# ChantalMP/RaDialog

Hardware: AMD Instinct MI355X
Metric: reports_per_sec (448px CXR encode + 160-tok prefill + 256-tok greedy decode) (higher is better)
Workload: dtype bf16; 1 GPU; configs[1]: per-GPU batch 1 BioViL-T(ResNet-50)+Q-Former encode 448px, Vicuna-7B prefill T=160, 256-token greedy decode (LoRA r=8 un-merged, hipGraph ; per_gpu_batch=1, global_batch=1, prompt_len=160, parallelism=dp1

## Files before the change

### radialog_amd/csrc/api.hip

```cpp
#include "rdx_ctx.h"

static std::string g_create_err;

int fail(rdx_ctx* c, int code, const char* fmt, ...) {
    char buf[512];
    va_list ap;
    va_start(ap, fmt);
    vsnprintf(buf, sizeof(buf), fmt, ap);
    va_end(ap);
    if (c) c->err = buf; else g_create_err = buf;
    return code;
}

const char* create_error() { return g_create_err.c_str(); }

int dalloc(rdx_ctx* c, void** p, size_t bytes) {
    if (bytes == 0) bytes = 16;
    hipError_t e = hipMalloc(p, bytes);
    if (e != hipSuccess) return fail(c, -3, "hipMalloc(%zu bytes) failed: %s", bytes, hipGetErrorString(e));
    c->allocs.push_back(*p);
    return 0;
}

extern "C" int rdx_create(rdx_ctx** out, int device_id, const rdx_config* cfg) {
// ... 4 lines not shown
    if (e != hipSuccess || ndev <= 0) return fail(nullptr, -2, "rdx_create: no HIP device (%s)", hipGetErrorString(e));
    if (device_id < 0 || device_id >= ndev) return fail(nullptr, -1, "rdx_create: device %d out of range (%d devices)", device_id, ndev);
    if (cfg->enable_llama) {
        if (cfg->hidden % cfg->heads || cfg->hidden / cfg->heads != 128)
            return fail(nullptr, -1, "rdx_create: Llama head_dim must be 128 (hidden %d / heads %d)", cfg->hidden, cfg->heads);
        if (cfg->hidden % 32 || cfg->inter % 32 || cfg->inter % 8 || cfg->qformer_dim % 32)
            return fail(nullptr, -1, "rdx_create: hidden/inter/qformer_dim must be multiples of 32");
        if (cfg->max_len % 32 || cfg->max_len <= 0 || cfg->max_len > 1536)
            return fail(nullptr, -1, "rdx_create: max_len must be a multiple of 32 in (0, 1536]");
        if (cfg->max_batch <= 0 || cfg->max_batch > RDX_MAX_ROWS) return fail(nullptr, -1, "rdx_create: max_batch must be in [1, %d]", RDX_MAX_ROWS);
        if (cfg->lora_r != 0 && cfg->lora_r != 8) return fail(nullptr, -1, "rdx_create: lora_r must be 0 or 8");
    }
    if (cfg->enable_vision) {
        if (cfg->q_hidden / cfg->q_heads != 64 || cfg->q_hidden % cfg->q_heads)
            return fail(nullptr, -1, "rdx_create: Q-Former head_dim must be 64");
    }
    if (cfg->enable_vision || cfg->enable_cls) {
        if (cfg->v_img % 4 || cfg->v_img < 32) return fail(nullptr, -1, "rdx_create: image size must be a multiple of 4, >= 32");
    }
    if (cfg->enable_cls) {
        if (cfg->enable_vision) return fail(nullptr, -1, "rdx_create: a classifier context has enable_vision = 0 (its projector differs)");
        if (cfg->cls_pool <= 0 || cfg->cls_hidden % 32 || cfg->cls_classes <= 0 || cfg->cls_classes > 16)
            return fail(nullptr, -1, "rdx_create: classifier needs pool > 0, hidden %% 32 == 0, 1..16 classes");
    }
    rdx_ctx* c = new rdx_ctx();
    c->cfg = *cfg;
    c->device = device_id;
    if (const char* e = getenv("RDX_FUSE_AO")) c->fuse_attn_oproj = atoi(e) != 0;
    if (const char* e = getenv("RDX_CHAIN")) c->chain_mlp = atoi(e) != 0;
    if (hipSetDevice(device_id) != hipSuccess || hipStreamCreateWithFlags(&c->stream, hipStreamNonBlocking) != hipSuccess) {
        delete c;
        return fail(nullptr, -2, "rdx_create: cannot create stream on device %d", device_id);
    }
    { const char* e = getenv("RDX_FLASH_MIN"); if (e) c->flash_min = atoi(e); }
    { const char* e = getenv("RDX_XS16"); if (e) c->xs16 = atoi(e) != 0; }
    { const char* e = getenv("RDX_PBLK"); if (e) c->prompt_blk = atoi(e) != 0; }
    { const char* e = getenv("RDX_BLK_DOWN"); c->blk_down = !(e && atoi(e) == 0); }
    { const char* e = getenv("RDX_PCONV_KSPLIT"); c->pconv_noks = e && atoi(e) == 0; }
    { const char* e = getenv("RDX_PCONV"); c->trunk_packed = !(e && atoi(e) == 0); }
    if (hipMalloc(&c->zero16, 64) == hipSuccess) { hipMemset(c->zero16, 0, 64); c->allocs.push_back(c->zero16); } else c->zero16 = nullptr;
    c->gemm_ws_floats = (size_t)16 << 20;
    if (hipMalloc((void**)&c->gemm_ws, c->gemm_ws_floats * sizeof(float)) != hipSuccess) { c->gemm_ws = nullptr; c->gemm_ws_floats = 0; }
    else c->allocs.push_back(c->gemm_ws);
    *out = c;
    return 0;
}

void rdx_comm_release(rdx_ctx* c);

extern "C" void rdx_destroy(rdx_ctx* c) {
    if (!c) return;
    hipSetDevice(c->device);
    hipStreamSynchronize(c->stream);
    rdx_comm_release(c);
    if (c->graph) hipGraphExecDestroy(c->graph);
    for (void* p : c->allocs) hipFree(p);
    hipStreamDestroy(c->stream);
    delete c;
}

extern "C" const char* rdx_last_error(rdx_ctx* c) { return c ? c->err.c_str() : g_create_err.c_str(); }

#ifndef RDX_BUILD_HASH
#define RDX_BUILD_HASH "unstamped"
#endif
extern "C" const char* rdx_build_hash(void) { return RDX_BUILD_HASH; }
// ... 230 lines not shown
        if (c->tens.count("v.pool.emb")) {
            const int Cv = f.v_b2v, Pn = v_grid(f) * v_grid(f);
            if (Cv % 32) return fail(c, -1, "ViT pooler needs b2v %% 32 == 0");
            c->pool_emb = R.t("v.pool.emb", (int64_t)2 * Pn * Cv);
            c->pool_ng = R.f("v.pool.norm_g", Cv); c->pool_nb = R.f("v.pool.norm_b", Cv);
            c->v_p1f = R.g("v.proj1f.w", f.v_proj, 2 * Cv); c->v_p1f_b = R.f("v.proj1f.b", f.v_proj);
            for (int i = 0; c->gemm.count(S("v.pool.%d.wqkv", i)); ++i) {
                PoolBlock pb;
                const std::string p = S("v.pool.%d.", i);
                pb.n1_g = R.f(p + "n1_g", Cv); pb.n1_b = R.f(p + "n1_b", Cv); pb.n2_g = R.f(p + "n2_g", Cv); pb.n2_b = R.f(p + "n2_b", Cv);
                pb.wqkv = R.g(p + "wqkv", 3 * Cv, Cv);
                pb.wo = R.g(p + "wo", Cv, Cv); pb.bo = R.f(p + "bo", Cv);
                pb.w1 = R.g(p + "w1", Cv, Cv); pb.b1 = R.f(p + "b1", Cv);
                pb.w2 = R.g(p + "w2", Cv, Cv); pb.b2 = R.f(p + "b2", Cv);
                c->pool.push_back(pb);
            }
        }
    }
    if (R.rc) return R.rc;
    c->finalized = true;
    return 0;
}

extern "C" int rdx_set_option(rdx_ctx* c, const char* name, int value) {
    if (!c || !name) return -1;
    if (!strcmp(name, "flash_min")) { c->flash_min = value; return 0; }
    if (!strcmp(name, "pconv")) { c->trunk_packed = value != 0; return 0; }
    if (!strcmp(name, "prompt_blk")) { c->prompt_blk = value != 0; return 0; }
    if (!strcmp(name, "xs16")) {
        c->xs16 = value != 0;
        if (c->graph) { hipGraphExecDestroy(c->graph); c->graph = nullptr; c->gkey = GraphKey(); }
        return 0;
    }
    return fail(c, -1, "rdx_set_option: unknown option '%s'", name);
}
```

### radialog_amd/csrc/api_debug.hip

```cpp
#include "rdx_ctx.h"
#include "../../include/rdx_hooks.h"
#include "../../include/rdx_enc_hooks.h"

extern "C" int rdx_attn_trace(rdx_ctx* c, int layer, long long* host) {
    if (!c || !c->finalized || c->cur_B <= 0 || !host) return fail(c, -1, "rdx_attn_trace: run a prefill first");
    HIPCHK(c, hipSetDevice(c->device));
    long long* dtr = nullptr;
    HIPCHK(c, hipMalloc(&dtr, 8 * sizeof(long long)));
    HIPCHK(c, hipMemsetAsync(dtr, 0, 8 * sizeof(long long), c->stream));
    DecAttnArgs at = dec_attn_args(c, layer);
    at.trace = dtr;
    launch_decode_attention(c->cfg.dtype, at, c->cur_B, c->stream);
    hipError_t e = hipStreamSynchronize(c->stream);
    if (e == hipSuccess) e = hipMemcpy(host, dtr, 8 * sizeof(long long), hipMemcpyDeviceToHost);
    hipFree(dtr);
    HIPCHK(c, e);
    return 0;
}

extern "C" int rdx_quant_test(rdx_ctx* c, const void* X, int M, int K, int groups, int mode, const void* norm_w, float eps, void* out8, float* scales) {
    if (!c || !X || !out8 || !scales || M <= 0 || K <= 0 || K % 128) return fail(c, -1, "rdx_quant_test: bad arguments (K %% 128 == 0)");
    if (mode == 0 && (groups < 1 || groups > 4)) return fail(c, -1, "rdx_quant_test: 1..4 K groups");
    if (mode == 1 && !norm_w) return fail(c, -1, "rdx_quant_test: mode 1 needs the norm weight");
    HIPCHK(c, hipSetDevice(c->device));
    if (mode == 0) launch_quant_rows(c->cfg.dtype, X, K, out8, scales, M, K, groups, c->stream);
    else launch_rmsnorm_fp8(c->cfg.dtype, X, norm_w, out8, scales, M, K, eps, c->stream);
    HIPCHK(c, hipStreamSynchronize(c->stream));
    HIPCHK(c, hipGetLastError());
    return 0;
}

extern "C" int rdx_gemv_trace(rdx_ctx* c, int what, int layer, long long* host, int max_tiles) {
    if (!c || !c->finalized || c->cur_B <= 0 || !host) return fail(c, -1, "rdx_gemv_trace: run a prefill first");
    HIPCHK(c, hipSetDevice(c->device));
    const rdx_config& f = c->cfg;
    const int H = f.hidden, B = c->cur_B;
    if (what == 7) {
        if (layer < 0 || layer >= f.layers) return fail(c, -1, "rdx_gemv_trace(7): layer %d of %d", layer, f.layers);
        if (c->cur_T + c->cur_steps + 1 > f.max_len || c->cur_T + c->cur_steps + 1 > f.max_pos)
            return fail(c, -1, "rdx_gemv_trace(7): no room for one more decode step in the KV cache");
        const int wgs = H / 16 + ((c->ll[0].wqkv.Npad + 15) / 16 + 3) / 4;
        if (wgs > max_tiles) return fail(c, -1, "rdx_gemv_trace(7): need room for %d workgroups", wgs);
        long long* dtr = nullptr;
        const size_t bytes = (size_t)max_tiles * 8 * sizeof(long long);
        HIPCHK(c, hipMalloc(&dtr, bytes));
        HIPCHK(c, hipMemsetAsync(dtr, 0, bytes, c->stream));
        c->chain_trace = dtr; c->chain_trace_layer = layer;
        const bool chained = decode_step_launch(c, nullptr, nullptr, 0);
        c->chain_trace = nullptr; c->chain_trace_layer = -1;
        c->cur_steps = std::max(c->cur_steps + 1, c->cur_max_new);
        hipError_t e = hipStreamSynchronize(c->stream);
        if (e == hipSuccess) e = hipMemcpy(host, dtr, bytes, hipMemcpyDeviceToHost);
        hipFree(dtr);
        HIPCHK(c, e);
        if (!chained) return fail(c, -1, "rdx_gemv_trace(7): the chained down -> QKV launch is not active in this configuration (batch > 2, RDX_CHAIN=0)");
        return 0;
    }
    const LlamaLayer& L = c->ll[layer];
    long long* dtr = nullptr;
    const size_t bytes = (size_t)max_tiles * 8 * sizeof(long long);
    HIPCHK(c, hipMalloc(&dtr, bytes));
    HIPCHK(c, hipMemsetAsync(dtr, 0, bytes, c->stream));
    GemmArgs a = unit_args(c, &L, what == 1 ? UNIT_GATE_UP : what == 2 ? UNIT_QKV : UNIT_DOWN, B);
    if (what != 1 && what != 2) { a.out = c->dqkv; a.resid = nullptr; a.ldr = 0; }
    if ((a.N + 15) / 16 > max_tiles) { hipFree(dtr); return fail(c, -1, "rdx_gemv_trace: need room for %d tiles", (a.N + 15) / 16); }
    a.trace = dtr;
    skinny(c, a, what == 1 ? EPI_SILU_MUL : EPI_NONE);
    hipError_t e = hipStreamSynchronize(c->stream);
    if (e == hipSuccess) e = hipMemcpy(host, dtr, bytes, hipMemcpyDeviceToHost);
// ... 464 lines not shown
```

### radialog_amd/csrc/api_llama.hip

```cpp
#include "rdx_ctx.h"

static int ensure_prefill_ws(rdx_ctx* c, size_t rows) {
    rows = (rows + 15) & ~(size_t)15;
    if (rows <= c->prefill_rows) return 0;
    const rdx_config& f = c->cfg;
    HIPCHK(c, hipStreamSynchronize(c->stream));
    c->prefill_rows = 0;
    dfree(c, c->px); dfree(c, c->pxn); dfree(c, c->pqkv); dfree(c, c->pq); dfree(c, c->patt); dfree(c, c->pgu); dfree(c, c->pxq); dfree(c, c->pxs); dfree(c, c->pslab);
    if (fp8_weights(c->ll[0].wqkv)) {
        ALLOC(c, c->pxq, rows * (size_t)std::max(f.hidden, f.inter));
        ALLOC(c, c->pxs, rows * 4 * sizeof(float));
    }
    ALLOC(c, c->px, rows * f.hidden * 2); ALLOC(c, c->pxn, rows * f.hidden * 2);
    ALLOC(c, c->pslab, (size_t)4 * std::min<size_t>(rows, 192) * f.hidden * sizeof(float));
    ALLOC(c, c->pqkv, rows * c->ld.qkv_ld * 2); ALLOC(c, c->pq, rows * f.hidden * 2);
    ALLOC(c, c->patt, rows * f.hidden * 2); ALLOC(c, c->pgu, rows * f.inter * 2);
    c->prefill_rows = rows;
    return 0;
}

static const char* const k_need_blk = "more than 32 decoder rows need hidden 4096 / inter 11008 (the row-block family)";

static void lm_head_and_greedy(rdx_ctx* c, const void* x, int B, void* logits, const int* out_step, long step_stride,
                               int advance) {
// ... 164 lines not shown
    for (int l = 0; l < c->cfg.layers; ++l) {
        const LlamaLayer* L = &c->ll[l];
        launch_xstat_blk8(dt, norm_in_front(c, blk8_unit(c, L, UNIT_QKV, B)), EPI_NONE, s);
        DecAttnArgs at = dec_attn_args(c, l);
        at.out_packed = 2;
        launch_decode_attention(dt, at, B, s);
        ksplit(blk8_unit(c, L, UNIT_O, B));
        launch_xstat_blk8(dt, norm_in_front(c, blk8_unit(c, L, UNIT_GATE_UP, B)), EPI_SILU_MUL, s);
        ksplit(blk8_unit(c, L, UNIT_DOWN, B));
    }
}

static void step_xs16(rdx_ctx* c, int B) {
    const int dt = c->cfg.dtype;
    hipStream_t s = c->stream;
    for (int l = 0; l < c->cfg.layers; ++l) {
        const LlamaLayer* L = &c->ll[l];
        launch_xstat16(dt, xs16_unit(c, L, UNIT_QKV, B), EPI_NONE, s);
        DecAttnArgs at = dec_attn_args(c, l);
        at.out_packed = 1;
        launch_decode_attention(dt, at, B, s);
        launch_xrow16(dt, xs16_unit(c, L, UNIT_O, B), s);
        launch_xstat16(dt, xs16_unit(c, L, UNIT_GATE_UP, B), EPI_SILU_MUL, s);
        launch_xrow16(dt, xs16_unit(c, L, UNIT_DOWN, B), s);
    }
}

static void attn_oproj(rdx_ctx* c, int l, int B) {
    const int dt = c->cfg.dtype;
    const LlamaLayer& L = c->ll[l];
    DecAttnArgs at = dec_attn_args(c, l);
    const GemmArgs ao = unit_args(c, &L, UNIT_O, B);
    if (c->fuse_attn_oproj && attn_oproj16_supported(c->ld, L.wo.N, L.wo.K, B)) {
        launch_attn_oproj16(dt, at, ao, B, c->d_ctr + (size_t)l * 256, c->d_err, c->stream);
        return;
    }
    const GemmArgs ap = ksplit_args(ao);
    const int kg = (B >= xs_min_rows() && c->kslab) ? xsplit32_groups(ap) : 0;
    at.out_packed = kg > 0 ? ap.xpacked : 0;
    launch_decode_attention(dt, at, B, c->stream);
    if (kg) launch_ksplit(c, ap);
    else skinny(c, ao, EPI_RESID);
}

static void step_generic(rdx_ctx* c, int B) {
    for (int l = 0; l < c->cfg.layers; ++l) {
        const LlamaLayer& L = c->ll[l];
        skinny(c, unit_args(c, &L, UNIT_QKV, B), EPI_NONE);
        attn_oproj(c, l, B);
        const bool split = down_split_ok(c, L, B);
        GemmArgs gu = unit_args(c, &L, UNIT_GATE_UP, B);
        gu.out_packed = split ? ksplit_args(unit_args(c, &L, UNIT_DOWN, B)).xpacked : 0;
        skinny(c, gu, EPI_SILU_MUL);
        launch_down(c, L, B, split);
    }
}

static void step_chained(rdx_ctx* c, int B, std::vector<hipEvent_t>* evs) {
    const rdx_config& f = c->cfg;
    hipStream_t s = c->stream;
    ChainArgs ca;
    memset(&ca, 0, sizeof(ca));
    ca.layers = c->d_clayers; ca.hidden = f.hidden; ca.inter = f.inter; ca.qkv_n = c->ll[0].wqkv.Npad; ca.qkv_ld = c->ld.qkv_ld; ca.B = B; ca.eps = f.rms_eps;
    ca.dx = c->dx; ca.dqkv = c->dqkv; ca.dgu = c->dgu; ca.ctr = c->d_cctr; ca.err = c->d_err; ca.naps = c->chain_naps;
    const LlamaLayer& L0 = c->ll[0];
    ca.w8 = (L0.wqkv.w8 && L0.wdown.w8 && f.hidden % 64 == 0 && f.inter % 64 == 0) ? 1 : 0;
    auto mark = [&] { if (evs) { hipEvent_t e; hipEventCreate(&e); hipEventRecord(e, s); evs->push_back(e); } };
    skinny(c, unit_args(c, &L0, UNIT_QKV, B), EPI_NONE);
    for (int l = 0; l < f.layers; ++l) {
        attn_oproj(c, l, B);
        skinny(c, unit_args(c, &c->ll[l], UNIT_GATE_UP, B), EPI_SILU_MUL);
        mark();
        ca.layer = l;
        ca.trace = l == c->chain_trace_layer ? c->chain_trace : nullptr;
        launch_decode_chain(f.dtype, ca, l + 1 < f.layers, s);
        mark();
    }
}

bool decode_step_launch(rdx_ctx* c, void* logits, const int* out_step, long step_stride, std::vector<hipEvent_t>* evs) {
    const int B = c->cur_B;
    const DecFamily fam = decode_family(c, B);
    switch (fam) {
    case DEC_UNSUPPORTED: c->unsupported = k_need_blk; return false;
    case DEC_BLK: step_blk(c, B); break;
    case DEC_BLK8: step_blk8(c, B); break;
    case DEC_XS16: step_xs16(c, B); break;
    case DEC_CHAINED: step_chained(c, B, evs); break;
    case DEC_GENERIC: step_generic(c, B); break;
    }
    lm_head_and_greedy(c, c->dx, B, logits, out_step, step_stride, 1);
    return fam == DEC_CHAINED;
}

extern "C" int rdx_decode_step(rdx_ctx* c, void* logits) {
    if (!c) return -1;
    if (!c->finalized || c->cur_B <= 0) return fail(c, -1, "rdx_decode_step: no prefill has run");
    if (c->cur_steps >= c->cur_max_new)
        return fail(c, -1, "rdx_decode_step: all %d tokens of this prompt (max_new) have been generated; run a new prefill", c->cur_max_new);
    if (c->cur_T + c->cur_steps > c->cfg.max_len || c->cur_T + c->cur_steps > c->cfg.max_pos)
        return fail(c, -1, "rdx_decode_step: KV cache full (%d prompt + %d generated slots of %d)", c->cur_T, c->cur_steps, c->cfg.max_len);
    HIPCHK(c, hipSetDevice(c->device));
    decode_step_launch(c, logits, nullptr, 0);
    ++c->cur_steps;
// ... 246 lines not shown
```

### radialog_amd/csrc/attn_body.h

```cpp
#pragma once
#include "rdx_common.h"
#include "rdx_kernels.h"
#include "handoff.h"

namespace rdx {

template <typename T>
__device__ __forceinline__ float rope_one(float x, float partner_signed, float c, float s) {
    return rnd<T>(rnd<T>(x * c) + rnd<T>(partner_signed * s));
}

__host__ __device__ inline size_t decode_attention_smem_floats(int waves, int max_len) { return (size_t)waves * 128 + 128 + max_len; }

template <int N> __device__ __forceinline__ float row_share(float v) { return dpp_mov<0x150 + N>(v); }

template <typename T> __device__ __forceinline__ float dot2(unsigned a, unsigned b, float c);
template <> __device__ __forceinline__ float dot2<bf16>(unsigned a, unsigned b, float c) {
    typedef __bf16 v2b __attribute__((ext_vector_type(2)));
    return __builtin_amdgcn_fdot2_f32_bf16(__builtin_bit_cast(v2b, a), __builtin_bit_cast(v2b, b), c, false);
}
template <> __device__ __forceinline__ float dot2<f16>(unsigned a, unsigned b, float c) {
    typedef _Float16 v2h __attribute__((ext_vector_type(2)));
    return __builtin_amdgcn_fdot2(__builtin_bit_cast(v2h, a), __builtin_bit_cast(v2h, b), c, false);
}

template <typename T, int WAVES, bool DED = (WAVES == 8), typename WaitFn = NoWait, bool V_EARLY_ = !DED, int KG_ = 0, bool COH = false>
__device__ __forceinline__ void decode_attention_body(const DecAttnArgs& a, const int h, const int b, float* dsm,
                                                      WaitFn wait_inputs = WaitFn()) {
    typedef typename Vec8<T>::type V8;
    constexpr int D = 128;
    constexpr int CW = DED ? WAVES - 1 : WAVES;
    constexpr int KG = KG_ ? KG_ : ((DED && WAVES == 8) ? 4 : 2);
    constexpr int VR = 4 * KG;
    constexpr int SPAN = CW * 4;
    constexpr bool V_EARLY = V_EARLY_;
    constexpr int KT = 2, VT = 4;
    const LlamaDims& d = a.d;
    const T* qkv = reinterpret_cast<const T*>(a.qkv);
    const T* lbq = reinterpret_cast<const T*>(a.lbq);
    const T* lbv = reinterpret_cast<const T*>(a.lbv);
    const T* cos_t = reinterpret_cast<const T*>(a.cos_t);
    const T* sin_t = reinterpret_cast<const T*>(a.sin_t);

    const int tid = threadIdx.x, lane = tid & 63, w = __builtin_amdgcn_readfirstlane(tid >> 6);
    float* part = dsm;
    T* qT = reinterpret_cast<T*>(dsm + WAVES * D);
    float* S = dsm + WAVES * D + D;

    const int jsub = lane >> 4, doct = lane & 15;
    const int g = lane >> 4, r = lane & 15;
    const int H = d.hidden;
    const T* x = qkv + (size_t)b * d.qkv_ld;
    T* kc = reinterpret_cast<T*>(a.kcache) + ((size_t)b * d.heads + h) * d.max_len * D;
    T* vc = reinterpret_cast<T*>(a.vcache) + ((size_t)b * d.heads + h) * d.max_len * D;
    const uint8_t* km = a.key_mask + (size_t)b * d.max_len;

    if (a.trace && h == 0 && b == 0 && tid == 0) a.trace[7] = (long long)__builtin_amdgcn_s_memrealtime();
    const int cw = DED ? w - 1 : w;
    const bool owns_rows = !DED || w > 0;
    u4 kr[KG][4], vr[VR];
    unsigned kmw[KG];
    constexpr int KG_LO = (KG + 1) / 2, VR_LO = 4 * KG_LO;
    auto load_k = [&](int u0, int u1, int limit) {
#pragma unroll
        for (int u = 0; u < KG; ++u) {
            const int gb = (u * CW + cw) * 16;
            if (u >= u0 && u < u1 && gb < limit) {
                const int j = min(gb + r, d.max_len - 1);
#pragma unroll
                for (int c = 0; c < 4; ++c) kr[u][c] = ldg16(kc + kperm(j, c * 32 + g * 8, d.k_perm));
                kmw[u] = *reinterpret_cast<const unsigned*>(km + min(gb + 4 * g, d.max_len - 4));
            }
        }
    };
    auto load_v = [&](int u0, int u1, int limit) {
#pragma unroll
        for (int u = 0; u < VR; ++u) {
            if (u >= u0 && u < u1 && (u & ~1) * SPAN + cw * 4 < limit) {
                const int j = min(u * SPAN + cw * 4 + jsub, d.max_len - 1);
                vr[u] = ldg16(vc + (size_t)j * D + doct * 8);
            }
        }
    };
    constexpr bool HAS_WAIT = !__is_same(WaitFn, NoWait);
    const int n0 = h * D + doct * 8;
    u4 nq, nk_, nv, ncos, nsin, naq, nav, nbq0, nbq1, nbv0, nbv1;
    auto load_newtok = [&]() {
        auto ldx = [&](const T* p) -> u4 {
            if (!COH) return ldg16(p);
            const unsigned long long lo = ld8_agent(p), hi = ld8_agent(p + 4);
            return (u4){(unsigned)lo, (unsigned)(lo >> 32), (unsigned)hi, (unsigned)(hi >> 32)};
        };
        nq = ldx(x + n0); nk_ = ldx(x + H + n0); nv = ldx(x + 2 * H + n0);
        const T* cs = reinterpret_cast<const T*>(a.cur_rope);
        const T* cp = cs ? cs + (size_t)b * 2 * D : cos_t + (size_t)a.pos[b] * D;
        const T* sp = cs ? cs + (size_t)b * 2 * D + D : sin_t + (size_t)a.pos[b] * D;
        ncos = ldg16(cp + doct * 8); nsin = ldg16(sp + doct * 8);
        if (d.lora_r == 8) {
            const int e0 = 2 * jsub;
            naq = ldx(x + 3 * H); nav = ldx(x + 3 * H + 8);
            nbq0 = ldg16(lbq + (size_t)(n0 + e0) * 8); nbq1 = ldg16(lbq + (size_t)(n0 + e0 + 1) * 8);
            nbv0 = ldg16(lbv + (size_t)(n0 + e0) * 8); nbv1 = ldg16(lbv + (size_t)(n0 + e0 + 1) * 8);
        }
    };
    if (!HAS_WAIT && w == 0) load_newtok();
    if (owns_rows) {
        load_k(0, KG_LO, 0x7fffffff);
        if (V_EARLY) load_v(0, VR_LO, 0x7fffffff);
    }
    const int slot = a.slot_b[b];
    const int nk = slot + 1;
    long long* trc = (a.trace && h == 0 && b == 0 && tid == 0) ? a.trace : nullptr;
#define ATT_T(i) do { if (trc) trc[i] = (long long)__builtin_amdgcn_s_memrealtime(); } while (0)
    ATT_T(0);
    wait_inputs();
    ATT_T(1);

    float s_new = 0.f;
    if (w == 0) {
        float q8n[8], k8[8], v8[8];
        if (HAS_WAIT) load_newtok();
        const V8 qv = as_vec8<T>(nq), kv = as_vec8<T>(nk_), vv = as_vec8<T>(nv), cv = as_vec8<T>(ncos), sv_ = as_vec8<T>(nsin);
#pragma unroll
        for (int e = 0; e < 8; ++e) { q8n[e] = tof<T>(qv[e]); k8[e] = tof<T>(kv[e]); v8[e] = tof<T>(vv[e]); }
        if (d.lora_r == 8) {
            const V8 aq = as_vec8<T>(naq), av = as_vec8<T>(nav);
            const V8 bq0 = as_vec8<T>(nbq0), bq1 = as_vec8<T>(nbq1), bv0 = as_vec8<T>(nbv0), bv1 = as_vec8<T>(nbv1);
            float sq0 = 0.f, sq1 = 0.f, sv0 = 0.f, sv1 = 0.f;
#pragma unroll
            for (int i = 0; i < 8; ++i) {
                sq0 += tof<T>(bq0[i]) * tof<T>(aq[i]); sq1 += tof<T>(bq1[i]) * tof<T>(aq[i]);
                sv0 += tof<T>(bv0[i]) * tof<T>(av[i]); sv1 += tof<T>(bv1[i]) * tof<T>(av[i]);
            }
            sq0 = rnd<T>(rnd<T>(sq0) * d.lora_scale); sq1 = rnd<T>(rnd<T>(sq1) * d.lora_scale);
            sv0 = rnd<T>(rnd<T>(sv0) * d.lora_scale); sv1 = rnd<T>(rnd<T>(sv1) * d.lora_scale);
#pragma unroll
            for (int e = 0; e < 8; ++e) {
                const int src = ((e >> 1) << 4) | doct;
                const float dq = __shfl((e & 1) ? sq1 : sq0, src, 64), dv = __shfl((e & 1) ? sv1 : sv0, src, 64);
                q8n[e] = rnd<T>(q8n[e] + dq);
                v8[e] = rnd<T>(v8[e] + dv);
            }
        }
        const bool lo = doct < 8;
#pragma unroll
// ... 174 lines not shown
```

### radialog_amd/csrc/chain.hip

```cpp
#include "rdx_common.h"
#include "rdx_kernels.h"
#include "attn_body.h"
#include "handoff.h"
#include "skinny_body.h"

namespace rdx {

constexpr int CH_WAVES = 16;
constexpr int CH_THREADS = CH_WAVES * 64;
constexpr int CH_MAXM = 2;

struct ChainGemm {
    const void* X; int ldx;
    const void* W;
    const void* resid; int ldr;
    void* out; int ldo;
    int M, N, K;
    const void* norm_w; float eps;
    const void* W8; const float* wscale;
};

template <typename T, int EPI, bool NORM, int SUB, int XL, typename WaitFn, int U = 4, bool RESID_EARLY = false, bool W8 = false>
__device__ __forceinline__ void chain_tile(const ChainGemm& a, const int wg, const int ntiles, unsigned char* smem, WaitFn wait_inputs,
                                           long long* trace = nullptr) {
    typedef typename Vec8<T>::type V8;
    constexpr int WPS = CH_WAVES / SUB;
    float* red = reinterpret_cast<float*>(smem);
    float* ssq = red + CH_WAVES * 256;
    float* rstd_s = ssq + CH_WAVES * CH_MAXM;
    T* xs = reinterpret_cast<T*>(rstd_s + 16);

    const int lane = threadIdx.x & 63, wa = __builtin_amdgcn_readfirstlane(threadIdx.x >> 6);
    const int sub = wa / WPS, w = wa - sub * WPS;
    const int tile = wg * SUB + sub;
    const int tile_c = min(tile, ntiles - 1);
    const int r = lane & 15, g = lane >> 4;
    const int K = a.K, KC = W8 ? (K >> 6) : (K >> 5);
    const int c0 = (KC * w) / WPS, c1 = (KC * (w + 1)) / WPS;
    const T* X = reinterpret_cast<const T*>(a.X);
    const u4* wbase = reinterpret_cast<const u4*>(W8 ? a.W8 : a.W) + (size_t)tile_c * KC * 64 + lane;
    const int clast = min(max(c1 - 1, c0), KC - 1);
    long long* trc = (trace && threadIdx.x == 0) ? trace : nullptr;
#define CH_T(i) do { if (trc) trc[i] = (long long)__builtin_amdgcn_s_memrealtime(); } while (0)
    CH_T(0);

    u4 wa_[U], wb_[U];
#pragma unroll
    for (int u = 0; u < U; ++u) wa_[u] = ldg16_nt(wbase + (size_t)min(c0 + u, clast) * 64);
#pragma unroll
    for (int u = 0; u < U; ++u) wb_[u] = ldg16_nt(wbase + (size_t)min(c0 + U + u, clast) * 64);
    if (trace) {
        if (threadIdx.x < 64) asm volatile("s_waitcnt vmcnt(%0)" :: "n"(2 * U - 1) : "memory");
        CH_T(5);
    }

    constexpr int QPT_E = EPI == EPI_SILU_MUL ? 2 : 4;
    unsigned long long rs8_early = 0ull;
    if (RESID_EARLY && EPI == EPI_RESID && (int)threadIdx.x < SUB * a.M * QPT_E) {
        const int so = threadIdx.x / (a.M * QPT_E), rem = threadIdx.x - so * (a.M * QPT_E);
        const int m = rem / QPT_E, q = rem - m * QPT_E;
        const int n = (wg * SUB + so) * 16 + q * 4;
        if (wg * SUB + so < ntiles && n < a.N) rs8_early = ld8_agent(reinterpret_cast<const T*>(a.resid) + (size_t)m * a.ldr + n);
    }

    wait_inputs();
    CH_T(3);

    const int K4 = K >> 2, total4 = a.M * K4;
    unsigned long long xr[XL];
#pragma unroll
    for (int i = 0; i < XL; ++i) {
        const int c = threadIdx.x + i * CH_THREADS;
        xr[i] = 0ull;
        if (c < total4) { const int m = c / K4, k4 = c - m * K4; xr[i] = ld8_agent(X + (size_t)m * a.ldx + (size_t)k4 * 4); }
    }
    if (NORM) {
        float ss[CH_MAXM];
#pragma unroll
        for (int m = 0; m < CH_MAXM; ++m) ss[m] = 0.f;
#pragma unroll
        for (int i = 0; i < XL; ++i) {
            const int c = threadIdx.x + i * CH_THREADS;
            float t = 0.f;
#pragma unroll
            for (int j = 0; j < 4; ++j) { const float f = tof<T>(from_bits16<T>((unsigned short)(xr[i] >> (16 * j)))); t += f * f; }
            const int m = c < total4 ? c / K4 : 0;
// ... 127 lines not shown
                float u = 0.f;
#pragma unroll
                for (int i = 0; i < WPS; ++i) u += red[(so * WPS + i) * 256 + m * 16 + 8 + q * 4 + j];
                if (W8) u *= a.wscale[t_o * 16 + 8 + q * 4 + j];
                pk |= (unsigned long long)bits16<T>(fromf<T>(swiglu<T>(v[j], u))) << (16 * j);
            }
            if (ok) st8_agent(out + (size_t)m * a.ldo + t_o * 8 + q * 4, pk);
        }
    }
    CH_T(7);
#undef CH_T
}

template <typename T, bool W8>
__global__ __launch_bounds__(CH_THREADS, 4) void decode_chain_k(ChainArgs ca) {
    extern __shared__ __attribute__((aligned(16))) unsigned char msm[];
    const ChainLayer& L = ca.layers[ca.layer];
    int* ctr = ca.ctr + (size_t)ca.layer * HO_CTR_INTS;
    const int H = ca.hidden, B = ca.B;
    long long* trace = ca.trace ? ca.trace + (size_t)blockIdx.x * 8 : nullptr;
    if ((int)blockIdx.x < ca.nwg_down) {
        ChainGemm g = {ca.dgu, ca.inter, L.wdown, ca.dx, H, ca.dx, H, B, H, ca.inter, nullptr, 0.f, L.wdown8, L.sdown};
        chain_tile<T, EPI_RESID, false, 1, 6, WaitSharded, 4, false, W8>(g, blockIdx.x, ca.nwg_down, msm, WaitSharded{ctr, 0, ca.err, ca.naps, nullptr}, trace);
        publish_sc1(ctr, blockIdx.x);
        if (trace && threadIdx.x == 0) trace[2] = (long long)__builtin_amdgcn_s_memrealtime();
        return;
    }
    const ChainLayer& Ln = ca.layers[ca.layer + 1];
    ChainGemm g = {ca.dx, H, Ln.wqkv, nullptr, 0, ca.dqkv, ca.qkv_ld, B, ca.qkv_n, H, Ln.attn_norm, ca.eps, Ln.wqkv8, Ln.sqkv};
    chain_tile<T, EPI_NONE, true, 4, 2, WaitSharded, W8 ? 4 : 8, false, W8>(g, blockIdx.x - ca.nwg_down, (ca.qkv_n + 15) / 16, msm,
                                                                             WaitSharded{ctr, ca.nwg_down, ca.err, ca.naps, nullptr}, trace);
}

template <typename T, bool W8>
__global__ __launch_bounds__(CH_THREADS, 4) void attn_oproj16_k(DecAttnArgs at, ChainGemm g, int n_attn, int ntiles, int* counter, int* err) {
    extern __shared__ __attribute__((aligned(16))) unsigned char msm[];
    if ((int)blockIdx.x < n_attn) {
        const int b = blockIdx.x / at.d.heads, h = blockIdx.x - b * at.d.heads;
        decode_attention_body<T, CH_WAVES, true, NoWait, true, 0, true>(at, h, b, reinterpret_cast<float*>(msm));
        publish_sc1(counter, blockIdx.x);
    } else {
        chain_tile<T, EPI_RESID, false, 2, 2, WaitSharded, W8 ? 4 : 8, true, W8>(g, blockIdx.x - n_attn, ntiles, msm, WaitSharded{counter, n_attn, err, 1, nullptr});
    }
}

bool attn_oproj16_supported(const LlamaDims& d, int N, int K, int B) {
    const int ntiles = (N + 15) / 16;
    return B <= CH_MAXM && d.head_dim == 128 && K % 32 == 0 && N % 4 == 0 && (size_t)B * K <= 8192 &&
           d.heads * B + (ntiles + 1) / 2 <= 256;
}

void launch_attn_oproj16(int dtype, const DecAttnArgs& a, const GemmArgs& ga, int B, int* counter, int* err, hipStream_t s) {
    const int n_attn = a.d.heads * B, ntiles = (ga.N + 15) / 16;
    const bool w8 = ga.W8 && ga.wscale && ga.K % 64 == 0;
    ChainGemm g = {ga.X, ga.ldx, ga.W, ga.resid, ga.ldr, ga.out, ga.ldo, ga.M, ga.N, ga.K, nullptr, 0.f, ga.W8, ga.wscale};
    const size_t sm_gemm = (size_t)(CH_WAVES * 256 + CH_WAVES * CH_MAXM + 16) * 4 + (size_t)B * ga.K * 2;
    const size_t sm_att = decode_attention_smem_floats(CH_WAVES, a.d.max_len) * sizeof(float);
    const size_t smem = sm_gemm > sm_att ? sm_gemm : sm_att;
    dim3 grid(n_attn + (ntiles + 1) / 2), block(CH_THREADS);
    RDX_DISPATCH_T(dtype, T, {
        if (w8) hipLaunchKernelGGL((attn_oproj16_k<T, true>), grid, block, smem, s, a, g, n_attn, ntiles, counter, err);
        else hipLaunchKernelGGL((attn_oproj16_k<T, false>), grid, block, smem, s, a, g, n_attn, ntiles, counter, err);
    });
}

bool chain_supported(const LlamaDims& d, int inter, int B) {
    if (B > CH_MAXM || d.head_dim != 128 || d.hidden % 32 || inter % 32 || d.hidden % 16) return false;
    const size_t stage = (size_t)B * (inter > d.hidden ? inter : d.hidden) * 2;
    return stage <= 48 * 1024 && inter % 4 == 0 && (size_t)B * d.hidden <= 8192 && (size_t)B * inter <= 24576;
}

size_t chain_ctr_ints(int layers) { return (size_t)layers * HO_CTR_INTS; }

void launch_decode_chain(int dtype, ChainArgs ca, bool with_next_qkv, hipStream_t s) {
    ca.nwg_down = ca.hidden / 16;
    const int nwg_qkv = with_next_qkv ? ((ca.qkv_n + 15) / 16 + 3) / 4 : 0;
    const int kmax = ca.inter > ca.hidden ? ca.inter : ca.hidden;
    const size_t sm_gemm = (size_t)(CH_WAVES * 256 + CH_WAVES * CH_MAXM + 16) * 4 + (size_t)ca.B * kmax * 2;
    const size_t smem = sm_gemm > (size_t)84 * 1024 ? sm_gemm : (size_t)84 * 1024;
    dim3 grid(ca.nwg_down + nwg_qkv), block(CH_THREADS);
    RDX_DISPATCH_T(dtype, T, {
        static DevOnce attr_set;
        if (attr_set.first()) {
            hipFuncSetAttribute((const void*)decode_chain_k<T, false>, hipFuncAttributeMaxDynamicSharedMemorySize, 100 * 1024);
            hipFuncSetAttribute((const void*)decode_chain_k<T, true>, hipFuncAttributeMaxDynamicSharedMemorySize, 100 * 1024);
        }
        if (ca.w8) hipLaunchKernelGGL((decode_chain_k<T, true>), grid, block, smem, s, ca);
        else hipLaunchKernelGGL((decode_chain_k<T, false>), grid, block, smem, s, ca);
    });
}

}
```

### radialog_amd/csrc/rdx_ctx.h

```cpp
#pragma once
#include <hip/hip_runtime.h>
#include <stdarg.h>
#include <stdio.h>
#include <stdlib.h>
#include <string.h>

#include <algorithm>
#include <map>
#include <string>
#include <vector>

#include "../../include/rdx.h"
#include "rdx_common.h"
#include "rdx_kernels.h"

using namespace rdx;

constexpr int RDX_MAX_ROWS = 128;

struct GemmW { void* w = nullptr; int N = 0, K = 0, Npad = 0; void* w8 = nullptr; float* scale = nullptr; };
struct RawW { void* p = nullptr; int64_t rows = 0, cols = 0; };

struct LlamaLayer {
    const void *attn_norm, *mlp_norm, *lora_bq, *lora_bv;
// ... 37 lines not shown
    std::map<std::string, RawW> tens;
    std::map<std::string, RawW> f32;

    std::vector<LlamaLayer> ll;
    const void *embed = nullptr, *final_norm = nullptr, *rope_cos = nullptr, *rope_sin = nullptr;
    GemmW lm_head, img_proj_w;
    const float* img_proj_b = nullptr;
    LlamaDims ld;
    void *kcache = nullptr, *vcache = nullptr;
    size_t kv_layer_elems = 0;
    uint8_t* key_mask = nullptr;
    int *d_img_pos = nullptr, *d_pos_ids = nullptr, *d_pos = nullptr, *d_slot = nullptr, *d_step = nullptr, *d_unf = nullptr;
    float* part_val = nullptr; int* part_idx = nullptr; int n_vtiles = 0;
    void *dx = nullptr, *dxn = nullptr, *dqkv = nullptr, *datt = nullptr, *dgu = nullptr;
    float* dxs = nullptr;
    void* pxq = nullptr; float* pxs = nullptr;
    std::string unsupported;
    float* kslab = nullptr;
    int pend_groups = 0;
    void *px = nullptr, *pxn = nullptr, *pqkv = nullptr, *pq = nullptr, *patt = nullptr, *pgu = nullptr, *pqe = nullptr, *pimg = nullptr;
    size_t prefill_rows = 0;
    float* pslab = nullptr;
    int cur_B = 0, cur_T = 0, cur_max_new = 0, cur_eos = -1, cur_pad = 0;
    int cur_steps = 0;
    int32_t* cur_tokens = nullptr;
    hipGraphExec_t graph = nullptr;
    bool fuse_attn_oproj = true;
    bool chain_mlp = true;
    bool xs16 = true;
    bool prompt_blk = true;
    bool blk_down = true;
    int chain_naps = 1;
    long long* chain_trace = nullptr; int chain_trace_layer = -1;
    GemmW cls_fc1, cls_fc2; const float *cls_fc1_b = nullptr, *cls_fc2_b = nullptr;
    void *cls_pooled = nullptr, *cls_h = nullptr, *cls_out = nullptr;
    void* zero16 = nullptr;
    void* d_cur_rope = nullptr;
    ChainLayer* d_clayers = nullptr; int* d_cctr = nullptr;
    int *d_ctr = nullptr, *d_err = nullptr;
    int flash_min = 512;
    bool pconv_noks = false;
    bool trunk_packed = true;
    bool ws_ok = false;
    float* gemm_ws = nullptr; size_t gemm_ws_floats = 0;
    GraphKey gkey;

    void* bm_logits = nullptr; float* bm_scores = nullptr; float* bm_cand_s = nullptr; int* bm_cand_i = nullptr;
    int *bm_tok = nullptr, *bm_src = nullptr; int32_t* bm_out = nullptr; void* bm_scratch = nullptr;
    size_t bm_scratch_bytes = 0; int bm_rows = 0, bm_new = 0;

    void* tf_ws = nullptr; size_t tf_bytes = 0;

    void* comm = nullptr; int comm_rank = 0, comm_world = 0;

    std::vector<QLayer> ql;
    const void* q_query_ln = nullptr;
    GemmW q_wkv; const float* q_bkv = nullptr; int n_cross = 0;
    GemmW v_conv1, v_b2v, v_p1, v_p2;
    const float *v_conv1_b = nullptr, *v_p1_b = nullptr, *v_p2_b = nullptr, *v_ln_g = nullptr, *v_ln_b = nullptr;
    std::vector<VBlock> vb;
    std::vector<PoolBlock> pool;
    const void* pool_emb = nullptr;
    const float *pool_ng = nullptr, *pool_nb = nullptr, *v_p1f_b = nullptr;
    GemmW v_p1f;
    float pool_eps = 1e-6f;
    int enc_batch = 0;
// ... 63 lines not shown
```

### radialog_amd/csrc/rdx_kernels.h

```cpp
#pragma once
#include <hip/hip_runtime.h>
#include <stdint.h>

namespace rdx {

enum Epilogue {
    EPI_NONE = 0,
    EPI_RELU = 1,
    EPI_GELU = 2,
    EPI_RESID = 3,
    EPI_SILU_MUL = 4,
    EPI_LOGITS = 5,
    EPI_RESID_RELU = 6,
};

struct GemmArgs {
    const void* X; int ldx;
    const void* W;
    const float* bias;
    const void* resid; int ldr;
    void* out; int ldo;
    int M, N, K;
    const void* norm_w; float eps;
    float* part_val; int* part_idx;
// ... 87 lines not shown
void launch_rmsnorm_blk_fp8(int dtype, void* x, const void* w, void* out8, float* xscale, int rows, int mtiles, float eps, const float* slab, int groups, hipStream_t s);
bool wsgemm_supported(const GemmArgs& a, const ConvGeom& cg, int epi);
void launch_wsgemm(int dtype, const GemmArgs& a, const ConvGeom& cg, int epi, const void* zero16, hipStream_t s);

bool pconv_supported(const PConvArgs& a, int taps, int stride, int epi);
bool launch_pconv(int dtype, PConvArgs a, int taps, int stride, int epi, bool rowout, hipStream_t s);
bool layernorm_packed_supported(int H);
void launch_layernorm_packed(int dtype, const void* x, const float* gamma, const float* beta, void* out, float* out_f32, int M, int H, float eps, hipStream_t s);
void launch_broadcast_packed(int dtype, const void* src, void* dst, int rows, int H, int B, hipStream_t s);
void launch_pack_rows(int dtype, const void* X, int ldx, void* P, int M, int C, hipStream_t s);
void launch_unpack_rows(int dtype, const void* P, void* X, int ldx, int M, int C, hipStream_t s);

bool stem_pool_supported(int stem_channels);
void launch_stem_pool(int dtype, const void* in, const void* Wp, const float* bias, void* out, int B, int Hp, int Hc, int Ho, int stem,
                      int packed_mt, hipStream_t s);

void launch_l2_bench(int mode, const void* buf, size_t bytes_per_wg, int shared, int reps, int wgs, unsigned* sink, hipStream_t s);

void launch_attention(int dtype, int head_dim, const AttnArgs& a, hipStream_t s);
bool flash_prefill_supported(int head_dim, const AttnArgs& a);
void launch_flash_prefill(int dtype, const AttnArgs& a, hipStream_t s);
void launch_rope_kv_prefill(int dtype, const LlamaDims& d, const void* qkv, const void* lora_bq, const void* lora_bv,
                            const void* cos_t, const void* sin_t, const int* pos_ids, void* qout, void* kcache,
                            void* vcache, int B, int T, int slot0, hipStream_t s);
void launch_k_unperm(const void* kc, void* out, size_t slabs, int max_len, int perm, hipStream_t s);
struct DecAttnArgs {
    LlamaDims d;
    const void *qkv, *lbq, *lbv, *cos_t, *sin_t;
    const void* cur_rope = nullptr;
    const int *pos, *slot_b;
    const uint8_t* key_mask;
    void *kcache, *vcache, *out;
    long long* trace = nullptr;
    int out_packed = 0;
    int out_mt = 2;
};
void launch_decode_attention(int dtype, const DecAttnArgs& a, int B, hipStream_t s);
struct ChainLayer { const void *wqkv, *wdown, *attn_norm;
                    const void *wqkv8, *wdown8; const float *sqkv, *sdown; };
struct ChainArgs {
    const ChainLayer* layers;
    int layer;
    int hidden, inter, qkv_n, qkv_ld, B;
    int w8;
    float eps;
    void *dx, *dqkv, *dgu;
    int* ctr;
    int* err;
    int naps;
    int nwg_down;
    long long* trace;
};
bool chain_supported(const LlamaDims& d, int inter, int B);
size_t chain_ctr_ints(int layers);
void launch_decode_chain(int dtype, ChainArgs ca, bool with_next_qkv, hipStream_t s);
bool attn_oproj16_supported(const LlamaDims& d, int N, int K, int B);
void launch_attn_oproj16(int dtype, const DecAttnArgs& a, const GemmArgs& g, int B, int* counter, int* err, hipStream_t s);

void launch_rmsnorm(int dtype, const void* x, const void* w, void* out, int rows, int H, float eps, hipStream_t s);
void launch_quant_rows(int dtype, const void* x, long ldx, void* out8, float* xscale, int rows, int K, int groups, hipStream_t s);
void launch_rmsnorm_fp8(int dtype, const void* x, const void* w, void* out8, float* xscale, int rows, int H, float eps, hipStream_t s);
void launch_rmsnorm_packed32_fp8(int dtype, void* x, const void* w, void* out8, float* xscale, int rows, int H, float eps, const float* slab,
                                 int groups, hipStream_t s);
bool gemm8_supported(const GemmArgs& a, int epi);
void launch_gemm8(int dtype, const GemmArgs& a, int epi, hipStream_t s);
void launch_rmsnorm_packed32(int dtype, void* x, const void* w, void* out, int rows, int H, float eps, int pack, const float* slab,
                             int groups, hipStream_t s);
void launch_layernorm(int dtype, const void* x, const float* gamma, const float* beta, void* out, float* out_f32,
                      int rows, int H, float eps, hipStream_t s);
void launch_layernorm_ex(int dtype, const void* x, long ldx, const float* gamma, const float* beta, const void* emb, int emb_rows,
                         void* out, long ldo, int rows, int H, float eps, hipStream_t s);
void launch_pool_gather(int dtype, const void* src, void* dst, int B, int L, int C, hipStream_t s);
void launch_pool_concat(int dtype, const void* patch, const void* tokens, void* dst, int B, int L, int C, hipStream_t s);
void launch_scramble_layernorm(int dtype, const void* pp_nhwc, const float* gamma, const float* beta, void* out,
                               float* out_f32, int B, int P, int C, float eps, hipStream_t s);
void launch_img_prep(int dtype, const float* img, void* out, int B, int S, int pad, int Hp, int Wp, hipStream_t s);
void launch_maxpool(int dtype, const void* in, void* out, int B, int H, int W, int C, hipStream_t s);
void launch_broadcast_rows(int dtype, const void* src, void* dst, int rows, int H, int B, hipStream_t s);
void launch_avgpool_flatten(int dtype, const void* in, void* out, int B, int G, int C, int pool, hipStream_t s);
void launch_to_f32(int dtype, const void* src, float* dst, size_t n, hipStream_t s);
void launch_from_f32(int dtype, const float* src, void* dst, size_t n, hipStream_t s);

void launch_prep_prompt(const int* ids, const int* mask_in, int B, int T, int img_id, int pad_id, int* img_pos,
                        int* pos_ids, uint8_t* key_mask, long km_bs, int* pos_next, int* slot_b, int* step_b,
                        int* unfinished, hipStream_t s);
void launch_prep_append(int B, int T_, int keep_len, int* img_pos, int* pos_ids, int* pos_next, int* slot_b, int* step_b,
                        int* unfinished, hipStream_t s);
void launch_embed_splice(int dtype, const int* ids, const int* img_pos, const void* embed, int vocab, const void* img_emb,
                         int n_img, void* out, int B, int T, int H, int use_img, hipStream_t s);
void launch_gather_last(int dtype, const void* x, void* out, int B, int T, int H, hipStream_t s);
// ... 14 lines not shown
```

Baseline: 1.514 reports/s.

## Prefetch gate/up weights into cache from idle CUs during fused attention+o_proj

Adds extra workgroups to the fused decode attention + o_proj launch, filling CUs that would otherwise sit idle. After a short delay they stream a slice of the next gate/up projection's weights (about 20 MiB by default at batch 1 with bf16 weights) so the following skinny GEMM finds them in cache. It also adds tracing hooks and option knobs for warm size, prefix and delay. The risk is that the warm loads compete with attention and o_proj for memory bandwidth, and the warmed lines may be evicted before the gate/up kernel runs.

Result: no change. 1.527 reports/s (median of 6 runs) (+0.9%).

```diff
diff --git a/radialog_amd/csrc/api.hip b/radialog_amd/csrc/api.hip
--- a/radialog_amd/csrc/api.hip
+++ b/radialog_amd/csrc/api.hip
@@ -60,6 +60,7 @@
         delete c;
         return fail(nullptr, -2, "rdx_create: cannot create stream on device %d", device_id);
     }
+    if (hipDeviceGetAttribute(&c->n_cus, hipDeviceAttributeMultiprocessorCount, device_id) != hipSuccess) c->n_cus = 0;
     { const char* e = getenv("RDX_FLASH_MIN"); if (e) c->flash_min = atoi(e); }
     { const char* e = getenv("RDX_XS16"); if (e) c->xs16 = atoi(e) != 0; }
     { const char* e = getenv("RDX_PBLK"); if (e) c->prompt_blk = atoi(e) != 0; }
@@ -356,5 +357,13 @@
         if (c->graph) { hipGraphExecDestroy(c->graph); c->graph = nullptr; c->gkey = GraphKey(); }
         return 0;
     }
+    int* warm = !strcmp(name, "attn_warm_kib") ? &c->attn_warm_kib : !strcmp(name, "attn_warm_prefix") ? &c->attn_warm_prefix :
+                !strcmp(name, "attn_warm_delay") ? &c->attn_warm_delay : nullptr;
+    if (warm) {
+        if (value < 0) return fail(c, -1, "rdx_set_option: %s must be >= 0", name);
+        *warm = value;
+        if (c->graph) { hipGraphExecDestroy(c->graph); c->graph = nullptr; c->gkey = GraphKey(); }
+        return 0;
+    }
     return fail(c, -1, "rdx_set_option: unknown option '%s'", name);
 }
diff --git a/radialog_amd/csrc/api_debug.hip b/radialog_amd/csrc/api_debug.hip
--- a/radialog_amd/csrc/api_debug.hip
+++ b/radialog_amd/csrc/api_debug.hip
@@ -35,6 +35,28 @@
     HIPCHK(c, hipSetDevice(c->device));
     const rdx_config& f = c->cfg;
     const int H = f.hidden, B = c->cur_B;
+    if (what == 8) {
+        if (layer < 0 || layer >= f.layers) return fail(c, -1, "rdx_gemv_trace(8): layer %d of %d", layer, f.layers);
+        if (c->cur_T + c->cur_steps + 1 > f.max_len || c->cur_T + c->cur_steps + 1 > f.max_pos)
+            return fail(c, -1, "rdx_gemv_trace(8): no room for one more decode step in the KV cache");
+        if (!(c->fuse_attn_oproj && attn_oproj16_supported(c->ld, H, H, B)) || decode_family(c, B) != DEC_CHAINED)
+            return fail(c, -1, "rdx_gemv_trace(8): the fused attention + o_proj launch is not active in this configuration (batch > 2, RDX_FUSE_AO=0, RDX_CHAIN=0)");
+        if (max_tiles < 256) return fail(c, -1, "rdx_gemv_trace(8): need room for 256 workgroups");
+        long long* dtr = nullptr;
+        const size_t bytes = (size_t)max_tiles * 8 * sizeof(long long);
+        HIPCHK(c, hipMalloc(&dtr, bytes));
+        HIPCHK(c, hipMemsetAsync(dtr, 0, bytes, c->stream));
+        const int gu_tiles = (c->ll[layer].wgu.Npad + 15) / 16;
+        c->ao_trace = dtr; c->ao_trace_layer = layer; c->ao_trace_gu = max_tiles >= 256 + gu_tiles ? dtr + (size_t)256 * 8 : nullptr;
+        decode_step_launch(c, nullptr, nullptr, 0);
+        c->ao_trace = nullptr; c->ao_trace_layer = -1; c->ao_trace_gu = nullptr;
+        c->cur_steps = std::max(c->cur_steps + 1, c->cur_max_new);
+        hipError_t e = hipStreamSynchronize(c->stream);
+        if (e == hipSuccess) e = hipMemcpy(host, dtr, bytes, hipMemcpyDeviceToHost);
+        hipFree(dtr);
+        HIPCHK(c, e);
+        return 0;
+    }
     if (what == 7) {
         if (layer < 0 || layer >= f.layers) return fail(c, -1, "rdx_gemv_trace(7): layer %d of %d", layer, f.layers);
         if (c->cur_T + c->cur_steps + 1 > f.max_len || c->cur_T + c->cur_steps + 1 > f.max_pos)
diff --git a/radialog_amd/csrc/api_llama.hip b/radialog_amd/csrc/api_llama.hip
--- a/radialog_amd/csrc/api_llama.hip
+++ b/radialog_amd/csrc/api_llama.hip
@@ -220,7 +220,11 @@
     DecAttnArgs at = dec_attn_args(c, l);
     const GemmArgs ao = unit_args(c, &L, UNIT_O, B);
     if (c->fuse_attn_oproj && attn_oproj16_supported(c->ld, L.wo.N, L.wo.K, B)) {
-        launch_attn_oproj16(dt, at, ao, B, c->d_ctr + (size_t)l * 256, c->d_err, c->stream);
+        const GemmArgs gu = unit_args(c, &L, UNIT_GATE_UP, B);
+        const int kib = c->attn_warm_kib >= 0 ? c->attn_warm_kib : (B == 1 && !(gu.W8 && gu.wscale)) ? 20 * 1024 : 0;
+        const AttnWarm aw = {kib, c->attn_warm_prefix, c->attn_warm_delay, c->n_cus};
+        launch_attn_oproj16(dt, at, ao, B, c->d_ctr + (size_t)l * 256, c->d_err, gu, aw,
+                            l == c->ao_trace_layer ? c->ao_trace : nullptr, c->stream);
         return;
     }
     const GemmArgs ap = ksplit_args(ao);
@@ -257,7 +261,9 @@
     skinny(c, unit_args(c, &L0, UNIT_QKV, B), EPI_NONE);
     for (int l = 0; l < f.layers; ++l) {
         attn_oproj(c, l, B);
-        skinny(c, unit_args(c, &c->ll[l], UNIT_GATE_UP, B), EPI_SILU_MUL);
+        GemmArgs gu = unit_args(c, &c->ll[l], UNIT_GATE_UP, B);
+        if (l == c->ao_trace_layer && c->ao_trace_gu) gu.trace = c->ao_trace_gu;
+        skinny(c, gu, EPI_SILU_MUL);
         mark();
         ca.layer = l;
         ca.trace = l == c->chain_trace_layer ? c->chain_trace : nullptr;
diff --git a/radialog_amd/csrc/attn_body.h b/radialog_amd/csrc/attn_body.h
--- a/radialog_amd/csrc/attn_body.h
+++ b/radialog_amd/csrc/attn_body.h
@@ -55,7 +55,7 @@
     T* vc = reinterpret_cast<T*>(a.vcache) + ((size_t)b * d.heads + h) * d.max_len * D;
     const uint8_t* km = a.key_mask + (size_t)b * d.max_len;
 
-    if (a.trace && h == 0 && b == 0 && tid == 0) a.trace[7] = (long long)__builtin_amdgcn_s_memrealtime();
+    if (a.trace && (a.trace_all || (h == 0 && b == 0)) && tid == 0) a.trace[7] = (long long)__builtin_amdgcn_s_memrealtime();
     const int cw = DED ? w - 1 : w;
     const bool owns_rows = !DED || w > 0;
     u4 kr[KG][4], vr[VR];
@@ -110,7 +110,7 @@
     }
     const int slot = a.slot_b[b];
     const int nk = slot + 1;
-    long long* trc = (a.trace && h == 0 && b == 0 && tid == 0) ? a.trace : nullptr;
+    long long* trc = (a.trace && (a.trace_all || (h == 0 && b == 0)) && tid == 0) ? a.trace : nullptr;
 #define ATT_T(i) do { if (trc) trc[i] = (long long)__builtin_amdgcn_s_memrealtime(); } while (0)
     ATT_T(0);
     wait_inputs();
diff --git a/radialog_amd/csrc/chain.hip b/radialog_amd/csrc/chain.hip
--- a/radialog_amd/csrc/chain.hip
+++ b/radialog_amd/csrc/chain.hip
@@ -52,6 +52,10 @@
     if (trace) {
         if (threadIdx.x < 64) asm volatile("s_waitcnt vmcnt(%0)" :: "n"(2 * U - 1) : "memory");
         CH_T(5);
+        if (RESID_EARLY) {
+            if (threadIdx.x < 64) asm volatile("s_waitcnt vmcnt(0)" ::: "memory");
+            CH_T(2);
+        }
     }
 
     constexpr int QPT_E = EPI == EPI_SILU_MUL ? 2 : 4;
@@ -245,15 +249,72 @@
                                                                              WaitSharded{ctr, ca.nwg_down, ca.err, ca.naps, nullptr}, trace);
 }
 
-template <typename T, bool W8>
-__global__ __launch_bounds__(CH_THREADS, 4) void attn_oproj16_k(DecAttnArgs at, ChainGemm g, int n_attn, int ntiles, int* counter, int* err) {
+struct WarmArgs {
+    const void* base; unsigned long long bytes;
+    int kc;
+    int kib;
+    int prefix;
+    int delay;
+    int first;
+};
+
+__device__ __forceinline__ void warm_role(const WarmArgs& wm, long long* trace) {
+    constexpr int WB = 8;
+    const int lane = threadIdx.x & 63, wa = __builtin_amdgcn_readfirstlane(threadIdx.x >> 6);
+    long long* trc = (trace && threadIdx.x == 0) ? trace : nullptr;
+    const long long t0 = (long long)__builtin_amdgcn_s_memrealtime();
+    if (trc) trc[0] = t0;
+    const int kc = wm.kc;
+    if (wm.base && wm.bytes >= 16 && kc > 0 && wm.kib > 0) {
+        const int x = blockIdx.x & 7;
+        const int bmin = wm.first + ((x - (wm.first & 7) + 8) & 7);
+        const int nx = ((int)gridDim.x - 1 - bmin) / 8 + 1, rank = ((int)blockIdx.x - bmin) >> 3;
+        const int p = max(1, wm.prefix > 0 ? min(wm.prefix, kc / 4) : kc / 4);
+        const long long gt = (long long)(wm.bytes / ((unsigned long long)kc * 1024));
+        const int wt = (int)min(gt, (long long)(wm.kib / (4 * p)));
+        const int items = wt > x ? ((wt - x + 7) / 8) * 4 * p : 0;
+        const int stride = nx * CH_WAVES;
+        const char* base = reinterpret_cast<const char*>(wm.base);
+        if (wm.delay > 0) {
+            if (wa == 0) while ((long long)__builtin_amdgcn_s_memrealtime() - t0 < (long long)wm.delay) __builtin_amdgcn_s_sleep(16);
+            __syncthreads();
+        }
+        if (trc) trc[1] = (long long)__builtin_amdgcn_s_memrealtime();
+        for (int it = rank * CH_WAVES + wa; it < items; it += WB * stride) {
+            u4 v[WB];
+#pragma unroll
+            for (int u = 0; u < WB; ++u) {
+                v[u] = (u4){0u, 0u, 0u, 0u};
+                const int e = it + u * stride;
+                if (e < items) {
+                    const int i = e / (4 * p), rem = e - i * 4 * p, sl = rem / p, q = rem - sl * p;
+                    const int chunk = min((kc * sl) / 4 + q, kc - 1);
+                    unsigned long long off = ((unsigned long long)(x + 8 * i) * kc + chunk) * 1024ull + (unsigned)lane * 16u;
+                    off = off + 16 <= wm.bytes ? off : wm.bytes - 16;
+                    v[u] = ldg16(base + off);
+                }
+            }
+#pragma unroll
+            for (int u = 0; u < WB; ++u) asm volatile("" :: "v"(v[u].x), "v"(v[u].y), "v"(v[u].z), "v"(v[u].w));
+        }
+        asm volatile("s_waitcnt vmcnt(0)" ::: "memory");
+    }
+    if (trc) { trc[2] = (long long)__builtin_amdgcn_s_memrealtime(); trc[7] = trc[2]; }
+}
+
+template <typename T, bool W8, bool TRACED>
+__global__ __launch_bounds__(CH_THREADS, 4) void attn_oproj16_k(DecAttnArgs at, ChainGemm g, int n_attn, int ntiles, int* counter, int* err, WarmArgs wm,
+                                                                long long* trace) {
     extern __shared__ __attribute__((aligned(16))) unsigned char msm[];
+    long long* trw = (TRACED && trace) ? trace + (size_t)blockIdx.x * 8 : nullptr;
+    if ((int)blockIdx.x >= wm.first) { warm_role(wm, trw); return; }
     if ((int)blockIdx.x < n_attn) {
         const int b = blockIdx.x / at.d.heads, h = blockIdx.x - b * at.d.heads;
+        if (trw) { at.trace = trw; at.trace_all = 1; }
         decode_attention_body<T, CH_WAVES, true, NoWait, true, 0, true>(at, h, b, reinterpret_cast<float*>(msm));
         publish_sc1(counter, blockIdx.x);
     } else {
-        chain_tile<T, EPI_RESID, false, 2, 2, WaitSharded, W8 ? 4 : 8, true, W8>(g, blockIdx.x - n_attn, ntiles, msm, WaitSharded{counter, n_attn, err, 1, nullptr});
+        chain_tile<T, EPI_RESID, false, 2, 2, WaitSharded, W8 ? 4 : 8, true, W8>(g, blockIdx.x - n_attn, ntiles, msm, WaitSharded{counter, n_attn, err, 1, nullptr}, trw);
     }
 }
 
@@ -263,17 +324,29 @@
            d.heads * B + (ntiles + 1) / 2 <= 256;
 }
 
-void launch_attn_oproj16(int dtype, const DecAttnArgs& a, const GemmArgs& ga, int B, int* counter, int* err, hipStream_t s) {
+void launch_attn_oproj16(int dtype, const DecAttnArgs& a, const GemmArgs& ga, int B, int* counter, int* err, const GemmArgs& warm, const AttnWarm& aw,
+                         long long* trace, hipStream_t s) {
     const int n_attn = a.d.heads * B, ntiles = (ga.N + 15) / 16;
     const bool w8 = ga.W8 && ga.wscale && ga.K % 64 == 0;
     ChainGemm g = {ga.X, ga.ldx, ga.W, ga.resid, ga.ldr, ga.out, ga.ldo, ga.M, ga.N, ga.K, nullptr, 0.f, ga.W8, ga.wscale};
     const size_t sm_gemm = (size_t)(CH_WAVES * 256 + CH_WAVES * CH_MAXM + 16) * 4 + (size_t)B * ga.K * 2;
     const size_t sm_att = decode_attention_smem_floats(CH_WAVES, a.d.max_len) * sizeof(float);
     const size_t smem = sm_gemm > sm_att ? sm_gemm : sm_att;
-    dim3 grid(n_attn + (ntiles + 1) / 2), block(CH_THREADS);
+    const int nwork = n_attn + (ntiles + 1) / 2;
+    const bool warm8 = warm.W8 && warm.wscale && warm.K % 64 == 0;
+    const void* wbase = warm8 ? warm.W8 : warm.W;
+    const int wkc = warm8 ? warm.K >> 6 : warm.K >> 5;
+    const unsigned long long wbytes = (unsigned long long)((warm.N + 15) / 16) * wkc * 1024ull;
+    int nwarm = (wbase && wkc > 0 && aw.kib > 0 && aw.cus > nwork) ? aw.cus - nwork : 0;
+    if (nwork + nwarm > 256) nwarm = 256 - nwork;
+    WarmArgs wm = {nwarm ? wbase : nullptr, nwarm ? wbytes : 0ull, wkc, nwarm ? aw.kib : 0, aw.prefix, aw.delay, nwork};
+    dim3 grid(nwork + nwarm), block(CH_THREADS);
     RDX_DISPATCH_T(dtype, T, {
-        if (w8) hipLaunchKernelGGL((attn_oproj16_k<T, true>), grid, block, smem, s, a, g, n_attn, ntiles, counter, err);
-        else hipLaunchKernelGGL((attn_oproj16_k<T, false>), grid, block, smem, s, a, g, n_attn, ntiles, counter, err);
+        if (trace) {
+            if (w8) hipLaunchKernelGGL((attn_oproj16_k<T, true, true>), grid, block, smem, s, a, g, n_attn, ntiles, counter, err, wm, trace);
+            else hipLaunchKernelGGL((attn_oproj16_k<T, false, true>), grid, block, smem, s, a, g, n_attn, ntiles, counter, err, wm, trace);
+        } else if (w8) hipLaunchKernelGGL((attn_oproj16_k<T, true, false>), grid, block, smem, s, a, g, n_attn, ntiles, counter, err, wm, trace);
+        else hipLaunchKernelGGL((attn_oproj16_k<T, false, false>), grid, block, smem, s, a, g, n_attn, ntiles, counter, err, wm, trace);
     });
 }
 
diff --git a/radialog_amd/csrc/rdx_ctx.h b/radialog_amd/csrc/rdx_ctx.h
--- a/radialog_amd/csrc/rdx_ctx.h
+++ b/radialog_amd/csrc/rdx_ctx.h
@@ -93,6 +93,10 @@
     bool blk_down = true;
     int chain_naps = 1;
     long long* chain_trace = nullptr; int chain_trace_layer = -1;
+    long long* ao_trace = nullptr; int ao_trace_layer = -1;
+    long long* ao_trace_gu = nullptr;
+    int attn_warm_kib = -1, attn_warm_prefix = 0, attn_warm_delay = 500;
+    int n_cus = 0;
     GemmW cls_fc1, cls_fc2; const float *cls_fc1_b = nullptr, *cls_fc2_b = nullptr;
     void *cls_pooled = nullptr, *cls_h = nullptr, *cls_out = nullptr;
     void* zero16 = nullptr;
diff --git a/radialog_amd/csrc/rdx_kernels.h b/radialog_amd/csrc/rdx_kernels.h
--- a/radialog_amd/csrc/rdx_kernels.h
+++ b/radialog_amd/csrc/rdx_kernels.h
@@ -143,6 +143,7 @@
     const uint8_t* key_mask;
     void *kcache, *vcache, *out;
     long long* trace = nullptr;
+    int trace_all = 0;
     int out_packed = 0;
     int out_mt = 2;
 };
@@ -166,7 +167,9 @@
 size_t chain_ctr_ints(int layers);
 void launch_decode_chain(int dtype, ChainArgs ca, bool with_next_qkv, hipStream_t s);
 bool attn_oproj16_supported(const LlamaDims& d, int N, int K, int B);
-void launch_attn_oproj16(int dtype, const DecAttnArgs& a, const GemmArgs& g, int B, int* counter, int* err, hipStream_t s);
+struct AttnWarm { int kib, prefix, delay, cus; };
+void launch_attn_oproj16(int dtype, const DecAttnArgs& a, const GemmArgs& g, int B, int* counter, int* err, const GemmArgs& warm, const AttnWarm& aw,
+                         long long* trace, hipStream_t s);
 
 void launch_rmsnorm(int dtype, const void* x, const void* w, void* out, int rows, int H, float eps, hipStream_t s);
 void launch_quant_rows(int dtype, const void* x, long ldx, void* out8, float* xscale, int rows, int K, int groups, hipStream_t s);
```
